# ORNL/DDStore

Hardware: NVIDIA H100
Metric: batch_fetch_GBps (higher is better)
Workload: dtype u8

## Files before the change

### ddstore_b200/csrc/kernels.cu

```cuda
#include <cuda_runtime.h>
#include <stdint.h>
#include <stdio.h>
#include <stdlib.h>
#include <string.h>

#include <algorithm>
#include <atomic>
#include <type_traits>

#include "kernels.h"

namespace {

thread_local char g_cuda_err[512] = "";
std::atomic<unsigned long long> g_launches{0};

#define CUDA_TRY(expr)                                                                                   \
    do {                                                                                                 \
        cudaError_t e__ = (expr);                                                                        \
        if (e__ != cudaSuccess) {                                                                        \
            snprintf(g_cuda_err, sizeof(g_cuda_err), "%s failed: %s (%s:%d)", #expr, cudaGetErrorString(e__), \
                     __FILE__, __LINE__);                                                                \
            return (int)e__ ? (int)e__ : -1;                                                             \
        }                                                                                                \
// ... 216 lines not shown
        if (code) {
            report(status, tag, idx[k], code);
            continue;
        }
        src[k] = s;
        nbytes[k] = count[k] * vp[k]->row_bytes;
    }
}

__device__ __forceinline__ int64_t warp_incl_scan(int64_t v, int lane) {
#pragma unroll
    for (int d = 1; d < 32; d <<= 1) {
        int64_t o = __shfl_up_sync(0xffffffffu, v, d);
        if (lane >= d) v += o;
    }
    return v;
}
__device__ __forceinline__ int64_t warp_sum(int64_t v) {
#pragma unroll
    for (int d = 16; d > 0; d >>= 1) v += __shfl_xor_sync(0xffffffffu, v, d);
    return v;
}

struct GatherArgs {
    ddsk_var_t var;
    const int64_t *starts;
    int64_t count;
    const uint64_t *req_src;
    const int64_t *req_dst;
    const uint32_t *seg_tab;
    PlanSrc plan;
    int64_t *total_out;
    int64_t nreq;
    char *dst;
    int64_t dst_cap;
    int64_t *offsets_out;
    unsigned long long *status;
    unsigned long long status_tag;
    unsigned int *counters;
    union {
        struct {
            char *mdst[DDSK_MAX_MULTI];
            int64_t mcap[DDSK_MAX_MULTI];
            int64_t *moffsets[DDSK_MAX_MULTI];
        };
        struct {
            int64_t pad_slot;
            uint64_t pad_bits;
            int pad_log2, pad_in_log2, pad_out_log2;
            int64_t *pad_lengths;
        };
    };
    int min_seg_chunks;
    int overlap, skip_wait;
    int wait1_valid, wait2_valid;
    unsigned int seq;
    unsigned int *ovl;
    int wait_plan;
    unsigned long long *plan_word;
    int64_t plan_tiles;
    unsigned int *tickets;
    unsigned long long *host_mirror;
    unsigned long long *dbg;
    const ddsk_push_t *push;
    int64_t push_nreq;
    unsigned long long push_step;
};

constexpr int64_t SEG_GRAIN = 16384;

struct Piece {
    uint64_t src;
    int64_t dpos;
    uint32_t n;
    uint32_t off;
};

template <int PCAP>
struct PlanView {
    uint32_t src_s, dst_s;
    __device__ __forceinline__ uint64_t s(int64_t i) const { return lds64(src_s + (uint32_t)i * 8u); }
    __device__ __forceinline__ int64_t d(int64_t i) const { return (int64_t)lds32(dst_s + (uint32_t)i * 4u); }
};
template <>
struct PlanView<0> {
    const uint64_t *src;
    const int64_t *dst;
    const uint32_t *seg_tab;
    __device__ __forceinline__ uint64_t s(int64_t i) const { return __ldcg(&src[i]); }
    __device__ __forceinline__ int64_t d(int64_t i) const { return __ldcg(&dst[i]); }
};

__device__ __forceinline__ void pad_lookup(const GatherArgs &a, int64_t idx, uint64_t &src, int64_t &payload) {
    const int64_t ix[1] = {idx};
    uint64_t s[1];
    int64_t nbytes[1];
    plan_many<1>(a.var, a.plan, ix, a.nreq, a.status, a.status_tag, s, nbytes);
    src = s[0];
    payload = min(nbytes[0], a.pad_slot);
}

__device__ __forceinline__ uint4 pad_pattern(uint64_t bits, int el) {
    uint32_t lo, hi;
    if (el == 0) lo = hi = (uint32_t)(bits & 0xFFu) * 0x01010101u;
    else if (el == 1) lo = hi = (uint32_t)(bits & 0xFFFFu) * 0x00010001u;
    else if (el == 2) lo = hi = (uint32_t)bits;
// ... 849 lines not shown
                over |= endv - vbase[v] > a.mcap[v];
            }
        if (PCAP > 0) over |= w.T > 0xFFFFFFFFll;
        if constexpr (CVT) {
            w.valign = true;
#pragma unroll
            for (int v = 0; v < DDSK_MAX_MULTI; v++) w.vb[v] = vbase[v];
        }
    }
    auto dst_of = [&](int64_t dpos) -> char * {
        if (FIXED && push) {
            int p = 0;
            for (int k = 1; k < w.push_n; k++)
                if (dpos >= push_rbase[k] * w.nb) p = k;
            return (char *)push_win[p] + push_dst_off + (dpos - push_rbase[p] * w.nb);
        }
        if (!multi) return a.dst + dpos;
        int64_t b = vbase[0];
        char *d = a.mdst[0];
#pragma unroll
        for (int k = 1; k < DDSK_MAX_MULTI; k++)
            if (dpos >= vbase[k]) {
                b = vbase[k];
                d = a.mdst[k];
            }
        return d + (dpos - b);
    };
    auto out_of = [&](int64_t dpos, int &code, uint32_t &lut) -> char * {
        if constexpr (CVT) {
            if (!multi) {
                code = code0;
                lut = lut_s + (uint32_t)c.lut_off[0];
                return a.dst + cvt_scale<NORM>(dpos, code0);
            }
            int64_t b = vbase[0];
            char *d = a.mdst[0];
            int cd = c.code[0], lo = c.lut_off[0];
#pragma unroll
            for (int k = 1; k < DDSK_MAX_MULTI; k++)
                if (dpos >= vbase[k]) {
                    b = vbase[k];
                    d = a.mdst[k];
                    cd = c.code[k];
                    lo = c.lut_off[k];
                }
            code = cd;
            lut = lut_s + (uint32_t)lo;
            return d + cvt_scale<NORM>(dpos - b, cd);
        } else {
            return nullptr;
        }
    };
    {
        if constexpr (PAD) {
            w.seg_bytes = ddsk_fixed_seg_bytes(w.T, w.nb, nwarps, a.min_seg_chunks, CH);
        } else {
        int64_t target = w.T / (nwarps * 8);
        const int64_t unit = (!FIXED && PCAP == 0) ? SEG_GRAIN : (int64_t)CH;
        target = max((int64_t)a.min_seg_chunks * CH, min(target, (int64_t)1 << 20));
        target = max(target, unit);
        if (FIXED && w.nb > 0 && w.nb <= target)
            w.seg_bytes = (target / w.nb) * w.nb;
        else
            w.seg_bytes = (target / unit) * unit;
        }
        w.nseg = w.T > 0 ? (w.T + w.seg_bytes - 1) / w.seg_bytes : 0;
    }
    if (over) {
        if (gwarp == 0 && lane == 0) report(a.status, a.status_tag, a.nreq, DDSK_CODE_CAPACITY);
        w.nseg = 0;
    }

    if (FIXED && !PAD && !push && (w.nb <= 0 || over)) {
        for (int64_t i = gwarp * 32 + lane; i < a.nreq; i += nwarps * 32) {
            uint64_t s;
            int code = dev_locate(a.var, a.starts[i], a.count, &s);
            if (code) report(a.status, a.status_tag, i, code);
        }
    }

    const uint32_t ring = smem_u32(smem_dyn) + (uint32_t)warp * (uint32_t)(S * STAGE);

    uint32_t issued = 0, consumed = 0;
    bool more = w.nseg > 0;
    while (true) {
        while (more && issued - consumed < (uint32_t)(S - 1)) {
            Piece pc;
            const uint32_t total = w.template next_group<STAGE>(a, lane, pc, pass_gate);
            if (total == 0) {
                more = false;
                break;
            }
            const uint32_t st = issued % S;
            const uint32_t bar = smem_u32(&full_bar[warp][st]);
            bulk_wait_read<1>();
            if (lane == 0) mbar_expect_tx(bar, total);
            __syncwarp();
            const uint32_t al = (uint32_t)(pc.src & 15u);
            desc[warp][st][lane].dpos = pc.dpos;
            desc[warp][st][lane].n = pc.n;
            desc[warp][st][lane].pack = pc.off | (al << 16);
            if (pc.n)
                tma_load_1d(ring + st * STAGE + pc.off, (const void *)(pc.src - al), (al + pc.n + 15u) & ~15u, bar);
            issued++;
        }
        if (consumed == issued) break;
        const uint32_t st = consumed % S;
        const uint32_t parity = (consumed / S) & 1u;
// ... 27 lines not shown
            const bool direct = my_code == 0 && my_n != 0 && (((uint32_t)(uint64_t)my_dst | my_n | (my_pack >> 16)) & 15u) == 0;
            if (direct) tma_store_1d(my_dst, ring + st * STAGE + (my_pack & 0xffffu), my_n);
            unsigned todo = __ballot_sync(0xffffffffu, my_n != 0 && !direct);
            while (todo) {
                const int j = __ffs(todo) - 1;
                todo &= todo - 1;
                const int64_t dpos = __shfl_sync(0xffffffffu, my_dpos, j);
                const uint32_t n = __shfl_sync(0xffffffffu, my_n, j);
                const uint32_t pk = __shfl_sync(0xffffffffu, my_pack, j);
                int code;
                uint32_t lut;
                char *const d = out_of(dpos, code, lut);
                const uint32_t s0 = ring + st * STAGE + (pk & 0xffffu);
                if constexpr (NORM) {
                    if (DDSK_CVT_IS_NORM(code)) {
                        norm_piece(c, multi, vbase, dpos, code, lut, d, s0 + (pk >> 16), n, lane);
                        continue;
                    }
                }
                switch (code) {
                case DDSK_CVT_F32_BF16: cvt_drain<DDSK_CVT_F32_BF16>(s0 + (pk >> 16), d, n, lut, lane); break;
                case DDSK_CVT_F32_F16: cvt_drain<DDSK_CVT_F32_F16>(s0 + (pk >> 16), d, n, lut, lane); break;
                case DDSK_CVT_F64_F32: cvt_drain<DDSK_CVT_F64_F32>(s0 + (pk >> 16), d, n, lut, lane); break;
                case DDSK_CVT_U8_LUT16: cvt_drain<DDSK_CVT_U8_LUT16>(s0 + (pk >> 16), d, n, lut, lane); break;
                case DDSK_CVT_U8_LUT32: cvt_drain<DDSK_CVT_U8_LUT32>(s0 + (pk >> 16), d, n, lut, lane); break;
                default: drain_chunk<CH>(s0, pk >> 16, d, n, lane); break;
                }
            }
        } else {
        char *const my_dst = dst_of(my_dpos);
        const bool direct = my_n != 0 && (((uint32_t)(uint64_t)my_dst | my_n | (my_pack >> 16)) & 15u) == 0;
        if (direct) tma_store_1d(my_dst, ring + st * STAGE + (my_pack & 0xffffu), my_n);
        unsigned todo = __ballot_sync(0xffffffffu, my_n != 0 && !direct);
        while (todo) {
            const int j = __ffs(todo) - 1;
            todo &= todo - 1;
            const int64_t dpos = __shfl_sync(0xffffffffu, my_dpos, j);
            const uint32_t n = __shfl_sync(0xffffffffu, my_n, j);
            const uint32_t pk = __shfl_sync(0xffffffffu, my_pack, j);
            drain_chunk<CH>(ring + st * STAGE + (pk & 0xffffu), pk >> 16, dst_of(dpos), n, lane);
        }
        }
        bulk_commit();
        __syncwarp();
        consumed++;
    }
    if (a.overlap || (FIXED && push)) {
        bulk_wait_all<0>();
        fence_proxy_async_global();
    } else {
        bulk_wait_read<0>();
    }
    __syncwarp();
    pass_gate();
    if (multi) {
        for (int64_t i = gwarp * 32 + lane; i < a.nreq + a.plan.nvars; i += nwarps * 32) {
            const int v = (int)(i / (a.plan.per_var + 1));
            const int64_t j = i - (int64_t)v * (a.plan.per_var + 1);
            if (v < a.plan.nvars && a.moffsets[v]) {
                const int64_t basev = w.pv.d((int64_t)v * a.plan.per_var);
                int64_t e = (v * a.plan.per_var + j == a.nreq) ? w.T : w.pv.d((int64_t)v * a.plan.per_var + j);
                if constexpr (CVT) a.moffsets[v][j] = cvt_scale<NORM>(e - basev, c.code[v]);
                else a.moffsets[v][j] = e - basev;
            }
        }
        if constexpr (CVT) {
            if (gwarp == 0 && lane == 0 && a.total_out) {
                int64_t t = 0;
#pragma unroll
                for (int v = 0; v < DDSK_MAX_MULTI; v++)
                    if (v < a.plan.nvars) t += cvt_scale<NORM>((v + 1 < a.plan.nvars ? vbase[v + 1] : w.T) - vbase[v], c.code[v]);
                *a.total_out = t;
            }
        }
    }
    if constexpr (PAD) {
        if (a.pad_lengths || w.nb == 0) {
            for (int64_t i = gwarp * 32 + lane; i < a.nreq; i += nwarps * 32) {
                uint64_t src;
                int64_t payload;
                pad_lookup(a, i, src, payload);
                if (a.pad_lengths) a.pad_lengths[i] = payload / a.var.row_bytes;
            }
        }
    }
    if (FIXED && a.offsets_out && !push) {
        if constexpr (CVT) {
            for (int64_t i = gwarp * 32 + lane; i <= a.nreq; i += nwarps * 32) a.offsets_out[i] = cvt_scale<NORM>(i * w.nb, code0);
        } else {
            for (int64_t i = gwarp * 32 + lane; i <= a.nreq; i += nwarps * 32) a.offsets_out[i] = i * w.nb;
        }
    }

    if (a.dbg && lane == 0) atomicMax(&a.dbg[blockIdx.x * 4 + 3], (unsigned long long)globaltimer_ns());
    if (a.overlap) {
        if (lane == 0) {
            __threadfence();
            const unsigned int slot = a.seq & 3u;
            const unsigned int done = atomicAdd(&a.ovl[slot], 1u);
            if (done == (unsigned int)(nwarps - 1)) {
                a.ovl[slot] = 0;
                a.ovl[8 + slot] = 0;
                if (a.wait_plan) a.plan_word[slot] = 0;
                if (a.wait1_valid) spin_until_done(a.ovl, a.seq - 1u, a.status, a.status_tag, a.nreq);
                __threadfence();
                st_release_u32(&a.ovl[4 + slot], a.seq);
            }
        }
    } else if (lane == 0) {
        if (FIXED && push) __threadfence_system(); else __threadfence();
        unsigned int done = atomicAdd(&a.counters[1], 1u);
        if (done == (unsigned int)(nwarps - 1)) {
            a.counters[0] = 0;
            a.counters[1] = 0;
            __threadfence();
            if (FIXED && push) {
                const ddsk_push_t *ps = a.push;
                for (int r = 0; r < ps->nranks; r++)
                    st_release_sys_u64((unsigned long long *)ps->win[r] + 8 + ps->me, a.push_step);
                const unsigned long long *hdr = (const unsigned long long *)ps->win[ps->me];
                const uint64_t t0 = globaltimer_ns();
                for (int r = 0; r < ps->nranks; r++)
                    while (ld_acquire_sys_u64(&hdr[8 + r]) < a.push_step) {
                        __nanosleep(200);
                        if (globaltimer_ns() - t0 > 30000000000ull) {
                            report(a.status, a.status_tag, a.nreq, DDSK_CODE_WATCHDOG);
                            __trap();
                        }
                    }
                const unsigned long long st = *(volatile const unsigned long long *)&hdr[3];
                if (st != DDSK_STATUS_OK) atomicMin(a.status, st | a.status_tag);
            }
            if (a.host_mirror) {
                a.host_mirror[0] = *(volatile unsigned long long *)a.status;
                a.host_mirror[1] = (unsigned long long)w.T;
                __threadfence_system();
            }
        }
    }
}

__global__ void __launch_bounds__(256) dds_small_get_kernel(const __grid_constant__ ddsk_var_t var, int64_t start, int64_t count,
                                                            char *__restrict__ dst, int64_t dst_cap,
                                                            volatile unsigned long long *flag, unsigned long long ticket) {
    uint64_t src = 0;
    const int code = dev_locate(var, start, count, &src);
    const int64_t n = code ? 0 : count * var.row_bytes;
    unsigned long long st = DDSK_STATUS_OK;
    if (code) st = (unsigned long long)code;
    else if (n > dst_cap) st = ((unsigned long long)1 << 8) | DDSK_CODE_CAPACITY;
    if (st == DDSK_STATUS_OK && n > 0) {
        const char *s = (const char *)src;
        if ((((uint64_t)s | (uint64_t)dst | (uint64_t)n) & 15u) == 0) {
            const uint4 *s4 = (const uint4 *)s;
            uint4 *d4 = (uint4 *)dst;
            for (int64_t i = threadIdx.x; i < (n >> 4); i += blockDim.x) d4[i] = s4[i];
        } else if ((((uint64_t)s | (uint64_t)dst | (uint64_t)n) & 3u) == 0) {
            const uint32_t *s1 = (const uint32_t *)s;
            uint32_t *d1 = (uint32_t *)dst;
            for (int64_t i = threadIdx.x; i < (n >> 2); i += blockDim.x) d1[i] = s1[i];
        } else {
            for (int64_t i = threadIdx.x; i < n; i += blockDim.x) dst[i] = s[i];
        }
    }
    __threadfence_system();
// ... 296 lines not shown
}

int geometry_for(bool fixed, int64_t request_bytes) {
    if (fixed) {
        if (g_geom_fixed_env >= 0) return g_geom_fixed_env;
        return request_bytes < 2048 ? kGeomSmall : kGeomLarge;
    }
    return g_geom_var_env >= 0 ? g_geom_var_env : kGeomVar;
}
int geometry_s_for(int64_t nreq) {
    if (nreq > kPlanSmemMax || nreq > g_plan_smem_default) return -1;
    if (g_geom_s_env >= 0 && kGeomsS[g_geom_s_env].pcap >= nreq) return g_geom_s_env;
    return nreq <= 4096 ? 0 : 1;
}

constexpr int smem_bytes_of(int nw, int s, int ch, int pcap) { return nw * s * (ch + 32) + (pcap ? pcap * 12 + 16 : 0); }
int static_smem_of(int nw, int s) { return nw * s * (8 + 32 * 16) + 16 * 8 + 64; }
int ctas_per_sm_for(int nw, int s, int ch, int pcap) {
    int per_sm = g_ctas_per_sm;
    while (per_sm > 1 && per_sm * (smem_bytes_of(nw, s, ch, pcap) + static_smem_of(nw, s) + 1024) > 227 * 1024) per_sm--;
    return per_sm;
}

bool cvt_has_norm(const ddsk_cvt_t *cvt) {
    for (int v = 0; v < DDSK_MAX_MULTI; v++)
        if (DDSK_CVT_IS_NORM(cvt->code[v])) return true;
    return false;
}

template <bool FIXED, int NW, int S, int CH, int PCAP, bool CVT = false, bool NORM = false, bool PAD = false>
int launch_gather_t(const GatherArgs &args_in, cudaStream_t stream, const ddsk_cvt_t *cvt = nullptr) {
    const int smem = smem_bytes_of(NW, S, CH, PCAP) + (CVT ? cvt->lut_bytes : 0);
    static std::atomic<unsigned long long> configured{0};
    auto kern = dds_gather_kernel<FIXED, NW, S, CH, PCAP, CVT, NORM, PAD>;
    int dev = 0;
    CUDA_TRY(cudaGetDevice(&dev));
    if (CVT) {
        if (dev >= 64 || !(configured.load() & (1ull << dev))) {
            cudaFuncAttributes fa;
            int optin = 0;
            CUDA_TRY(cudaFuncGetAttributes(&fa, kern));
            CUDA_TRY(cudaDeviceGetAttribute(&optin, cudaDevAttrMaxSharedMemoryPerBlockOptin, dev));
            const int most = std::min(smem_bytes_of(NW, S, CH, PCAP) + DDSK_MAX_MULTI * 1024, optin - (int)fa.sharedSizeBytes);
            CUDA_TRY(cudaFuncSetAttribute(kern, cudaFuncAttributeMaxDynamicSharedMemorySize, most));
            if (dev < 64) configured.fetch_or(1ull << dev);
        }
    } else if (dev >= 64 || !(configured.load() & (1ull << dev))) {
        CUDA_TRY(cudaFuncSetAttribute(kern, cudaFuncAttributeMaxDynamicSharedMemorySize, smem));
        if (dev < 64) configured.fetch_or(1ull << dev);
    }
    const int per_sm = ctas_per_sm_for(NW, S, CH, PCAP);
    GatherArgs args = args_in;
    args.dbg = g_dbg ? g_dbg + (size_t)(args.overlap ? (args.seq & 1u) : 0u) * kDbgRegion : nullptr;
    cudaLaunchConfig_t cfg = {};
    cfg.gridDim = dim3((unsigned)(g_sms * per_sm));
    cfg.blockDim = dim3(NW * 32);
    cfg.dynamicSmemBytes = smem;
    cfg.stream = stream;
    cudaLaunchAttribute attr[1];
    attr[0].id = cudaLaunchAttributeProgrammaticStreamSerialization;
    attr[0].val.programmaticStreamSerializationAllowed = g_pdl ? 1 : 0;
    cfg.attrs = attr;
    cfg.numAttrs = 1;
    if constexpr (CVT) {
        CUDA_TRY(cudaLaunchKernelEx(&cfg, kern, args, *cvt));
    } else {
        CUDA_TRY(cudaLaunchKernelEx(&cfg, kern, args, NoCvt{0}));
    }
    g_launches++;
    return 0;
}

template <int NW, int S, int CH, int PCAP>
bool cvt_s_fits_t(int lut_bytes) {
    cudaFuncAttributes fa;
    int dev = 0, optin = 0;
    if (cudaGetDevice(&dev) != cudaSuccess || cudaFuncGetAttributes(&fa, dds_gather_kernel<false, NW, S, CH, PCAP, true>) != cudaSuccess ||
        cudaDeviceGetAttribute(&optin, cudaDevAttrMaxSharedMemoryPerBlockOptin, dev) != cudaSuccess) {
        (void)cudaGetLastError();
        return false;
    }
    return smem_bytes_of(NW, S, CH, PCAP) + lut_bytes + (int)fa.sharedSizeBytes <= optin;
}

thread_local const void *g_l2_base = nullptr;
thread_local size_t g_l2_bytes = 0;

template <typename... KArgs, typename... Args>
int launch_pdl(void (*kern)(KArgs...), dim3 grid, dim3 block, cudaStream_t st, Args... args) {
    cudaLaunchConfig_t cfg = {};
    cfg.gridDim = grid;
    cfg.blockDim = block;
    cfg.dynamicSmemBytes = 0;
    cfg.stream = st;
    cudaLaunchAttribute attr[2];
    attr[0].id = cudaLaunchAttributeProgrammaticStreamSerialization;
    attr[0].val.programmaticStreamSerializationAllowed = g_pdl ? 1 : 0;
    cfg.attrs = attr;
    cfg.numAttrs = 1;
    if (g_l2_base && g_l2_bytes && g_l2_persist) {
        attr[1].id = cudaLaunchAttributeAccessPolicyWindow;
        attr[1].val.accessPolicyWindow.base_ptr = const_cast<void *>(g_l2_base);
        attr[1].val.accessPolicyWindow.num_bytes = g_l2_bytes;
        attr[1].val.accessPolicyWindow.hitRatio = 1.0f;
        attr[1].val.accessPolicyWindow.hitProp = cudaAccessPropertyPersisting;
        attr[1].val.accessPolicyWindow.missProp = cudaAccessPropertyStreaming;
        cfg.numAttrs = 2;
    }
// ... 372 lines not shown
```

### ddstore_b200/csrc/kernels.h

```cpp
#ifndef DDSK_KERNELS_H
#define DDSK_KERNELS_H

#include <stdint.h>

#ifdef __cplusplus
extern "C" {
#endif

#define DDSK_MAX_RANKS 64
#define DDSK_MAX_MULTI 4

typedef struct ddsk_var {
    const void *bases[DDSK_MAX_RANKS];
    int64_t lenlist[DDSK_MAX_RANKS];
    int64_t row_bytes;
    int32_t nranks;
    int32_t pad_;
} ddsk_var_t;

#define DDSK_STATUS_OK 0xFFFFFFFFFFFFFFFFull
#define DDSK_STATUS_ORD_SHIFT 48
#define DDSK_STATUS_REQ_MASK 0xFFFFFFFFFFull
#define DDSK_CODE_START 2
#define DDSK_CODE_COUNT 3
// ... 45 lines not shown
#define DDSK_CVT_PLAIN_IN_LOG2(c) ((c) == DDSK_CVT_F64_F32 ? 3 : ((c) == DDSK_CVT_F32_BF16 || (c) == DDSK_CVT_F32_F16) ? 2 : 0)
#define DDSK_CVT_PLAIN_OUT_LOG2(c) ((c) == DDSK_CVT_NONE ? 0 : ((c) == DDSK_CVT_F64_F32 || (c) == DDSK_CVT_U8_LUT32) ? 2 : 1)
#define DDSK_CVT_IN_LOG2(c) \
    (DDSK_CVT_IS_NORM(c) ? ((c) == DDSK_CVT_NORM_F64_F32 ? 3 : (c) >= DDSK_CVT_NORM_U8_F32 ? 0 : 2) : DDSK_CVT_PLAIN_IN_LOG2(c))
#define DDSK_CVT_OUT_LOG2(c)                                                                                              \
    (DDSK_CVT_IS_NORM(c) ? (((c) == DDSK_CVT_NORM_F32_F32 || (c) == DDSK_CVT_NORM_F64_F32 || (c) == DDSK_CVT_NORM_U8_F32) ? 2 : 1) \
                         : DDSK_CVT_PLAIN_OUT_LOG2(c))
typedef struct ddsk_cvt {
    int32_t code[DDSK_MAX_MULTI];
    int32_t lut_off[DDSK_MAX_MULTI];
    int32_t lut_bytes;
    int32_t pad_;
    uint32_t lut[DDSK_MAX_MULTI * 256];
    const float *norm[DDSK_MAX_MULTI];
    int32_t nchan[DDSK_MAX_MULTI];
    int32_t inner[DDSK_MAX_MULTI];
} ddsk_cvt_t;

int ddsk_gather_fixed(const ddsk_var_t *var, const int64_t *starts_dev, int64_t count, int64_t nreq, void *dst_dev,
                      int64_t dst_capacity, int64_t *offsets_dev_or_null, const ddsk_scratch_t *scr, int flags,
                      const ddsk_cvt_t *cvt, void *stream);

typedef struct ddsk_index {
    const int64_t *starts, *counts;
    const int64_t *sample_ids;
    const int64_t *table;
    int64_t nsamples;
} ddsk_index_t;

int ddsk_gather_var(const ddsk_var_t *var, const ddsk_index_t *index, int64_t nreq, void *dst_dev,
                    int64_t dst_capacity, int64_t *offsets_dev_or_null, ddsk_scratch_t *scr, int flags,
                    const ddsk_cvt_t *cvt, void *stream);
int ddsk_var_uses_scratch(int64_t nreq, int64_t dst_capacity, const ddsk_cvt_t *cvt);
int64_t ddsk_plan_smem_max(void);

int ddsk_gather_padded(const ddsk_var_t *var, const ddsk_index_t *index, int64_t nreq, int64_t max_rows, uint64_t pad_bits,
                       int pad_log2, int64_t *lengths, void *dst_dev, const ddsk_scratch_t *scr, int flags,
                       const ddsk_cvt_t *cvt, void *stream);

#if defined(__CUDACC__)
#define DDSK_HD __host__ __device__
#else
#define DDSK_HD
#endif

static inline DDSK_HD int64_t ddsk_fixed_seg_bytes(int64_t T, int64_t nb, int64_t nwarps, int64_t min_chunks, int64_t ch) {
    int64_t target = T / (nwarps * 8);
    if (target > ((int64_t)1 << 20)) target = (int64_t)1 << 20;
    if (target < min_chunks * ch) target = min_chunks * ch;
    if (target < ch) target = ch;
    return (nb > 0 && nb <= target) ? (target / nb) * nb : (target / ch) * ch;
}

typedef struct ddsk_pad_cut {
    int64_t pay_src, pay_len;
    int64_t pay_dst;
    int64_t pad_dst, pad_len;
} ddsk_pad_cut_t;
static inline DDSK_HD ddsk_pad_cut_t ddsk_pad_cut(int64_t i, int64_t payload, int64_t slot, int64_t lo, int64_t hi,
                                                  int in_log2, int out_log2) {
    ddsk_pad_cut_t c;
    const int64_t base = i * slot;
    const int64_t pe = payload < hi ? payload : hi;
    const int64_t ps = lo < pe ? lo : pe;
    const int64_t qs = lo > payload ? lo : payload;
    c.pay_src = base + ps;
    c.pay_len = pe - ps;
    c.pay_dst = ((base + ps) >> in_log2) << out_log2;
    c.pad_dst = ((base + qs) >> in_log2) << out_log2;
    c.pad_len = qs < hi ? ((hi - qs) >> in_log2) << out_log2 : 0;
    return c;
}

typedef struct ddsk_multi {
    int nvars;
    const ddsk_var_t *vars_dev;
    const int64_t *table[DDSK_MAX_MULTI];
    int64_t nsamples[DDSK_MAX_MULTI];
    void *dst[DDSK_MAX_MULTI];
    int64_t cap[DDSK_MAX_MULTI];
    int64_t *offsets[DDSK_MAX_MULTI];
} ddsk_multi_t;
int ddsk_gather_multi(const ddsk_multi_t *m, const int64_t *sample_ids_dev, int64_t nreq, ddsk_scratch_t *scr, int flags,
                      const ddsk_cvt_t *cvt, void *stream);

#define DDSK_PUSH_HDR_BYTES 4096
typedef struct ddsk_push {
    int32_t nranks, me;
    unsigned char *win[DDSK_MAX_RANKS];
    int64_t idx_off[2], dst_off[2];
    int64_t max_requests, max_bytes;
} ddsk_push_t;
int ddsk_gather_push(const ddsk_var_t *var, const ddsk_push_t *push_host, const ddsk_push_t *push_dev,
                     const int64_t *starts_dev, int64_t count, int64_t nreq, unsigned long long step,
                     const ddsk_scratch_t *scr, void *stream);

int ddsk_small_get(const ddsk_var_t *var, int64_t start, int64_t count, void *dst, int64_t dst_capacity,
                   unsigned long long *flag_dev, unsigned long long ticket, void *stream);

int ddsk_synth_fill(void *base_dev, int64_t first_global_row, int64_t nrows, int64_t disp, int itemsize, uint64_t seed,
                    void *stream);

typedef struct ddsk_mailbox {
    unsigned long long seq_head;
    int64_t start, count;
    uint64_t dst;
// ... 33 lines not shown
```

### ddstore_b200/csrc/store.cpp

```cpp
#include <cuda_runtime_api.h>
#include <sched.h>
#include <sys/random.h>
#include <unistd.h>

#include <algorithm>
#include <atomic>
#include <condition_variable>
#include <mutex>
#include <thread>
#include <cstdio>
#include <cstdlib>
#include <cstring>
#include <ctime>
#include <map>
#include <set>
#include <string>
#include <vector>

#include "ddstore_b200.h"
#include "internal.h"
#include "kernels.h"
#include "vmm.h"


// ... 1053 lines not shown
        if ((spins & 0xFFFF) == 0xFFFF) {
            cudaError_t q = cudaStreamQuery(s->db_stream);
            if (q != cudaErrorNotReady && q != cudaSuccess) {
                s->db_alive = false;
                return cuda_fail(q, "doorbell kernel");
            }
        }
#if defined(__x86_64__)
        __builtin_ia32_pause();
#endif
    }
    std::atomic_thread_fence(std::memory_order_acquire);
    const int code = (int)(r & 0xFFu);
    const int64_t n = code ? 0 : (count > 0 ? count * v->kv.row_bytes : 0);
    if (!dst_dev && n > 0) memcpy(dst, s->h_small + kSmallIdx * 16, (size_t)n);
    if (total_bytes) *total_bytes = n;
    if (!code) {
        if (bad_index) *bad_index = -1;
        return DDS_OK;
    }
    return decode_status_word(code == DDSK_CODE_CAPACITY ? (((unsigned long long)1 << 8) | DDSK_CODE_CAPACITY)
                                                          : (unsigned long long)code, bad_index);
}

static int small_get(dds_store_t *s, Var *v, int64_t start, int64_t count, void *dst, int64_t cap, bool dst_dev,
                     int64_t *total_bytes, int64_t *bad_index) {
    if (s->db_enabled && v->id >= 0) return doorbell_get(s, v, start, count, dst, cap, dst_dev, total_bytes, bad_index);
    cudaStream_t st = s->stream;
    volatile unsigned long long *flag = s->h_status;
    const unsigned long long ticket = ++s->small_ticket;
    void *d_dst = dst_dev ? dst : (void *)(s->d_small + kSmallIdx * 16);
    if (ddsk_small_get(&v->kv, start, count, d_dst, cap, s->scr.host_mirror, ticket, st))
        return fail(DDS_ERR_CUDA, ddsk_last_cuda_error());
    for (unsigned spins = 0; flag[2] != ticket; spins++) {
        if ((spins & 0x3FFF) == 0x3FFF) {
            cudaError_t q = cudaStreamQuery(st);
            if (q != cudaErrorNotReady) {
                if (q != cudaSuccess) return cuda_fail(q, "dds_small_get_kernel");
                if (flag[2] != ticket) return fail(DDS_ERR_CUDA, "small get: the kernel finished without publishing its ticket");
            }
        }
#if defined(__x86_64__)
        __builtin_ia32_pause();
#endif
    }
    std::atomic_thread_fence(std::memory_order_acquire);
    const unsigned long long stw = flag[0];
    const int64_t n = (int64_t)flag[1];
    if (!dst_dev && stw == DDSK_STATUS_OK && n > 0) memcpy(dst, s->h_small + kSmallIdx * 16, (size_t)n);
    if (total_bytes) *total_bytes = n;
    return decode_status_word(stw, bad_index);
}

static int stage_indices(dds_store_t *s, const int64_t *starts, const int64_t *counts, int64_t nreq, bool idx_dev,
                         cudaStream_t st, const int64_t **d_starts, const int64_t **d_counts) {
    if (idx_dev) return DDS_OK;
    if (nreq <= kSmallIdx) {
        int64_t *hs = (int64_t *)s->h_small, *hc = hs + kSmallIdx;
        memcpy(hs, starts, (size_t)nreq * 8);
        *d_starts = (const int64_t *)s->d_small;
        if (counts) {
            memcpy(hc, counts, (size_t)nreq * 8);
            *d_counts = (const int64_t *)s->d_small + kSmallIdx;
        }
        return DDS_OK;
    }
    if (int rc = ensure_idx(s, nreq)) return rc;
    CU(cudaMemcpyAsync(s->d_starts, starts, (size_t)nreq * 8, cudaMemcpyHostToDevice, st));
    *d_starts = s->d_starts;
    if (counts) {
        CU(cudaMemcpyAsync(s->d_counts, counts, (size_t)nreq * 8, cudaMemcpyHostToDevice, st));
        *d_counts = s->d_counts;
    }
    return DDS_OK;
}

static int batch_impl(dds_store_t *s, Var *v, bool by_sample, const int64_t *starts, const int64_t *counts,
                      int64_t fixed_count, int64_t nreq, void *dst, int64_t dst_capacity, int64_t *dst_offsets,
                      unsigned flags, void *cuda_stream, int64_t *total_bytes, int64_t *bad_index,
                      const ddsk_cvt_t *cvt = nullptr) {
    if (nreq < 0 || dst_capacity < 0) return fail(DDS_ERR_ARG, "negative nreq or capacity");
    if (nreq > 0 && !starts) return fail(DDS_ERR_ARG, "null starts / sample ids");
    const bool idx_dev = flags & DDS_IDX_ON_DEVICE, dst_dev = flags & DDS_DST_ON_DEVICE;
    const bool no_sync = flags & DDS_NO_SYNC;
    if (no_sync && !(idx_dev && dst_dev)) return fail(DDS_ERR_ARG, "async batches need device indices and a device destination");
    CU(cudaSetDevice(s->device));
    cudaStream_t st = cuda_stream ? (cudaStream_t)cuda_stream : s->stream;
    const bool chain = s->pending && no_sync && st == s->pending_stream;
    if (s->pending && !chain) {
        if (int rc = drain_pending(s)) return rc;
    }
    const int64_t R = v->kv.row_bytes;
    const bool fixed = !by_sample && counts == nullptr;
    const int64_t rows = v->lenlist.empty() ? 0 : v->lenlist.back();
    auto req_bytes = [&](int64_t c) { return c > 0 && c <= rows ? c * R : (int64_t)0; };
    const int64_t nb_fixed = fixed ? req_bytes(fixed_count) : 0;

    if (nreq == 0) {
        if (dst_offsets) {
            int64_t z = 0;
            if (dst_dev) CU(cudaMemcpyAsync(dst_offsets, &z, 8, cudaMemcpyHostToDevice, st));
            else dst_offsets[0] = 0;
            if (dst_dev) CU(cudaStreamSynchronize(st));
        }
        note_empty_async(s, no_sync);
        return DDS_OK;
    }

    if (fixed && nreq == 1 && !idx_dev && !no_sync && !cuda_stream && !dst_offsets && !cvt) {
        const int64_t need = nb_fixed;
        if (need <= (dst_dev ? (int64_t)(1 << 20) : kSmallOut) && (dst || need == 0))
            return small_get(s, v, starts[0], fixed_count, dst, dst_dev ? dst_capacity : std::min(dst_capacity, kSmallOut), dst_dev,
                             total_bytes, bad_index);
    }

    const int64_t *d_starts = starts, *d_counts = counts;
    if (int rc = stage_indices(s, starts, !fixed && !by_sample ? counts : nullptr, nreq, idx_dev, st, &d_starts, &d_counts))
        return rc;

    int64_t upper = -1;
    if (fixed)
        upper = sat_mul(nreq, nb_fixed);
    else if (!idx_dev && !by_sample) {
        upper = 0;
        for (int64_t i = 0; i < nreq; i++) upper = sat_add(upper, req_bytes(counts[i]));
    } else if (!idx_dev && by_sample && !v->h_tab_count.empty()) {
        upper = 0;
        for (int64_t i = 0; i < nreq; i++) {
            const int64_t id = starts[i];
            if (id >= 0 && id < v->nsamples) upper = sat_add(upper, req_bytes(v->h_tab_count[(size_t)id]));
        }
    }

    void *d_dst = dst;
    int64_t cap = dst_capacity;
    bool small_out = false;
    if (!dst_dev) {
        int64_t need = upper >= 0 ? std::min(upper, dst_capacity) : dst_capacity;
        if (need <= kSmallOut) {
// ... 782 lines not shown
```

### ddstore_b200/store.py

```python
import ctypes as C

import numpy as np

from . import _capi
from .comm import as_dds_comm

_NP_OK = {np.dtype(np.int32), np.dtype(np.int64), np.dtype(np.uint8), np.dtype(np.float32),
          np.dtype(np.float64), np.dtype(np.bool_)}
_TORCH_OK = {"torch.int32", "torch.int64", "torch.uint8", "torch.float32", "torch.float64", "torch.bool"}
_TORCH_HALF = {"torch.bfloat16", "torch.float16"}

_CVT_CODES = {("float32", "bfloat16"): _capi.CVT_F32_BF16, ("float32", "float16"): _capi.CVT_F32_F16,
              ("float64", "float32"): _capi.CVT_F64_F32, ("uint8", "bfloat16"): _capi.CVT_U8_LUT16,
              ("uint8", "float16"): _capi.CVT_U8_LUT16, ("uint8", "float32"): _capi.CVT_U8_LUT32}
_NORM_CODES = {("float32", "float32"): _capi.CVT_NORM_F32_F32, ("float32", "bfloat16"): _capi.CVT_NORM_F32_BF16,
               ("float32", "float16"): _capi.CVT_NORM_F32_F16, ("float64", "float32"): _capi.CVT_NORM_F64_F32,
               ("uint8", "float32"): _capi.CVT_NORM_U8_F32, ("uint8", "bfloat16"): _capi.CVT_NORM_U8_BF16,
               ("uint8", "float16"): _capi.CVT_NORM_U8_F16}
_U8_NORM = (_capi.CVT_NORM_U8_F32, _capi.CVT_NORM_U8_BF16, _capi.CVT_NORM_U8_F16)
_default_luts = {}


def _dtype_name(dt):
    s = str(dt)
# ... 70 lines not shown
    elif dtype.is_floating_point:
        v = float(value)
        t = torch.tensor([v], dtype=dtype)
        if math.isfinite(v) and not bool(torch.isfinite(t).all()):
            raise ValueError(f"pad_value {value!r} overflows {dtype}")
    else:
        if isinstance(value, float) and not value.is_integer():
            raise ValueError(f"pad_value {value!r} is not an integer ({dtype})")
        iv, info = int(value), torch.iinfo(dtype)
        if not info.min <= iv <= info.max:
            raise ValueError(f"pad_value {value!r} is outside the range of {dtype}")
        t = torch.tensor([iv], dtype=dtype)
    n = t.element_size()
    return int(t.view(getattr(torch, _INT_VIEW[n])).item()) & ((1 << (8 * n)) - 1)


def _lut_bits(t):
    import torch
    t = t.detach().reshape(-1).cpu().contiguous()
    return t.view(torch.int16 if t.element_size() == 2 else torch.int32).numpy().copy()


class _Buf:

    def __init__(self, arr, writable=False, half_ok=False):
        self.keep = arr
        if isinstance(arr, np.ndarray):
            assert arr.flags.c_contiguous
            if arr.dtype not in _NP_OK:
                raise NotImplementedError
            self.ptr, self.on_device = arr.ctypes.data, 0
            self.shape, self.itemsize, self.size = arr.shape, arr.dtype.itemsize, arr.size
        elif hasattr(arr, "data_ptr") and hasattr(arr, "element_size"):
            assert arr.is_contiguous()
            if str(arr.dtype) not in _TORCH_OK and not (half_ok and str(arr.dtype) in _TORCH_HALF):
                raise NotImplementedError
            self.ptr, self.on_device = arr.data_ptr(), 1 if arr.is_cuda else 0
            self.shape, self.itemsize, self.size = tuple(arr.shape), arr.element_size(), arr.numel()
        elif hasattr(arr, "__cuda_array_interface__"):
            cai = arr.__cuda_array_interface__
            if cai.get("strides") is not None:
                raise ValueError("device array must be C-contiguous")
            dt = np.dtype(cai["typestr"])
            if dt not in _NP_OK:
                raise NotImplementedError
            self.ptr, self.on_device = cai["data"][0], 1
            self.shape, self.itemsize = tuple(cai["shape"]), dt.itemsize
            self.size = int(np.prod(self.shape, dtype=np.int64))
        else:
            raise TypeError(f"unsupported array type {type(arr).__name__}")
        self.nbytes = self.size * self.itemsize


class _DevMem:

    def __init__(self, ptr, nbytes):
        self.__cuda_array_interface__ = {"shape": (int(nbytes),), "typestr": "|u1", "data": (int(ptr), False), "version": 2}


def _i64(x):
    return np.ascontiguousarray(x, dtype=np.int64)


class PyDDStore:
    def __init__(self, comm=None, method=0, device=None):
        self._L = _capi.lib()
        self._comm = as_dds_comm(comm)
        self._h = self._L.dds_create(self._comm.handle, -1 if device is None else int(device), int(method))
        if not self._h:
            raise RuntimeError(_capi.last_error())
        self.rank, self.size = self._L.dds_rank(self._h), self._L.dds_size(self._h)
        self._itemsize = {}
        self._cname = {}
        self._rowbytes = {}
        self.last_bad_index = -1

    def add(self, name, arr):
        b = _Buf(arr)
        nrows = b.shape[0]
        disp = b.size // b.shape[0] if b.shape[0] else int(np.prod(b.shape[1:], dtype=np.int64))
        _capi.raise_for(self._L.dds_add(self._h, name.encode(), b.ptr, nrows, disp, b.itemsize, b.on_device))

    def get(self, name, arr, start=0):
        cn = self._cname.get(name)
        if cn is None:
            cn = self._cname[name] = name.encode()
        if type(arr) is np.ndarray:
            assert arr.flags.c_contiguous
            if arr.dtype not in _NP_OK:
                raise NotImplementedError
            rc = self._L.dds_get(self._h, cn, int(start), arr.shape[0], arr.dtype.itemsize, arr.ctypes.data, 0)
        else:
            b = _Buf(arr, writable=True)
            rc = self._L.dds_get(self._h, cn, int(start), b.shape[0], b.itemsize, b.ptr, b.on_device)
        if rc:
            _capi.raise_for(rc)

    def epoch_begin(self):
        _capi.raise_for(self._L.dds_epoch_begin(self._h))

    def epoch_end(self):
        _capi.raise_for(self._L.dds_epoch_end(self._h))

    def free(self):
        if self._h:
            self._itemsize.clear()
            _capi.raise_for(self._L.dds_free(self._h))

    def init(self, name, nrows, disp, itemsize=1):
        _capi.raise_for(self._L.dds_init(self._h, name.encode(), int(nrows), int(disp), int(itemsize)))

    def update(self, name, arr, offset, stream=None, wait=True):
        b = _Buf(arr)
        if wait:
            rc = self._L.dds_update(self._h, name.encode(), b.ptr, b.shape[0], int(offset), b.itemsize, b.on_device)
        else:
            rc = self._L.dds_update_async(self._h, name.encode(), b.ptr, b.shape[0], int(offset), b.itemsize,
                                          b.on_device, self._stream_arg(stream))
        _capi.raise_for(rc)

    def ingest(self, name, arr, offset):
        b = _Buf(arr)
        if b.on_device:
            raise ValueError("ingest takes host arrays (use update for device arrays)")
        _capi.raise_for(self._L.dds_ingest(self._h, name.encode(), b.ptr, b.shape[0], int(offset), b.itemsize))

    def ingest_wait(self):
        _capi.raise_for(self._L.dds_ingest_wait(self._h))

    def get_batch(self, name, starts, counts=None, out=None, count=None, offsets=None, stream=None, wait=True,
                  overlap=False, src_dtype=None, lut=None, normalize=False, pad_rows=None, pad_value=0, lengths=None):
        if out is None:
            raise ValueError("get_batch needs an `out` buffer (like get(), it never allocates)")
        if pad_rows is not None:
            if counts is None:
                raise ValueError("pad_rows needs counts (there is no fixed-count padded batch)")
            if count is not None or offsets is not None:
                raise ValueError("a padded batch takes neither `count` nor `offsets`")
        cv = lut_keep = None
        if normalize and src_dtype is None:
            raise ValueError("normalize=True needs src_dtype")
        if src_dtype is not None:
            cv, lut_keep = _conversion(src_dtype, getattr(out, "dtype", None), lut, normalize)
        else:
            itemsize = self._itemsize.get(name)
            if itemsize is None:
                itemsize = self._itemsize[name] = self.query(name)["itemsize"]
        ob = _Buf(out, writable=True, half_ok=cv is not None or pad_rows is not None)
        s_dev = hasattr(starts, "data_ptr") and getattr(starts, "is_cuda", False)
        if s_dev:
            nreq = starts.numel()
            sp = starts.data_ptr()
            cp = counts.data_ptr() if counts is not None else None
            keep = (starts, counts)
        else:
            sa = _i64(starts)
            nreq = sa.size
            sp = sa.ctypes.data
            ca = _i64(counts) if counts is not None else None
            cp = ca.ctypes.data if ca is not None else None
            keep = (sa, ca)
        flags = (_capi.IDX_ON_DEVICE if s_dev else 0) | (_capi.DST_ON_DEVICE if ob.on_device else 0)
        if not wait:
            flags |= _capi.NO_SYNC | (_capi.OVERLAP if overlap else 0)
        if pad_rows is not None:
            return self._padded(name, False, sp, cp, nreq, out, ob, cv, pad_rows, pad_value, lengths, flags, stream,
                                (keep, lut_keep))
        op = None
        if offsets is not None:
            fb = _Buf(offsets, writable=True)
            if fb.on_device != ob.on_device or fb.itemsize != 8 or fb.size < nreq + 1:
                raise ValueError("offsets must be int64[len(starts)+1] with the same residency as out")
            op = fb.ptr
        total, bad = C.c_int64(0), C.c_int64(-1)
        if cv is None:
            rc = self._L.dds_get_batch(self._h, name.encode(), sp, cp, 1 if count is None else int(count), nreq,
                                       itemsize, ob.ptr, ob.nbytes, op, flags,
                                       self._stream_arg(stream), C.byref(total), C.byref(bad))
        else:
            rc = self._L.dds_get_batch_convert(self._h, name.encode(), sp, cp, 1 if count is None else int(count), nreq,
                                               ob.ptr, ob.nbytes, op, flags, self._stream_arg(stream), C.byref(cv),
                                               C.byref(total), C.byref(bad))
        del keep, lut_keep
        self.last_bad_index = bad.value
# ... 208 lines not shown
```

Baseline: 1466.

## Right-size fixed-batch grid, per-CTA completion counting, and a fast Python path

For fixed-count batches the host now works out the segment size and a reduced CTA count from the batch shape and passes the segment size to the kernel, so small batches no longer launch a full grid. The completion counter is now bumped once per CTA after a __syncthreads rather than once per warp, and only warps that have tail work pass the gate. The host side skips redundant cudaSetDevice calls, and the Python get_batch gains a fast path for async device batches that bypasses argument validation. The risks are correctness of the gate and counter logic with fewer CTAs, and a fast path that does less validation.

After: 1469, median of 6. Within noise of the previous version (+0.2%).

```diff
diff --git a/ddstore_b200/csrc/kernels.cu b/ddstore_b200/csrc/kernels.cu
--- a/ddstore_b200/csrc/kernels.cu
+++ b/ddstore_b200/csrc/kernels.cu
@@ -292,6 +292,7 @@
         };
     };
     int min_seg_chunks;
+    int64_t fixed_seg;
     int overlap, skip_wait;
     int wait1_valid, wait2_valid;
     unsigned int seq;
@@ -1247,8 +1248,8 @@
         }
     };
     {
-        if constexpr (PAD) {
-            w.seg_bytes = ddsk_fixed_seg_bytes(w.T, w.nb, nwarps, a.min_seg_chunks, CH);
+        if (FIXED && !push) {
+            w.seg_bytes = a.fixed_seg;
         } else {
         int64_t target = w.T / (nwarps * 8);
         const int64_t unit = (!FIXED && PCAP == 0) ? SEG_GRAIN : (int64_t)CH;
@@ -1382,7 +1383,13 @@
         bulk_wait_read<0>();
     }
     __syncwarp();
-    pass_gate();
+    {
+        bool tail = false;
+        if (multi) tail = gwarp * 32 < a.nreq + a.plan.nvars;
+        if (PAD && a.pad_lengths) tail = gwarp * 32 < a.nreq;
+        if (FIXED && a.offsets_out && !push) tail = gwarp * 32 <= a.nreq;
+        if (tail) pass_gate();
+    }
     if (multi) {
         for (int64_t i = gwarp * 32 + lane; i < a.nreq + a.plan.nvars; i += nwarps * 32) {
             const int v = (int)(i / (a.plan.per_var + 1));
@@ -1423,12 +1430,15 @@
     }
 
     if (a.dbg && lane == 0) atomicMax(&a.dbg[blockIdx.x * 4 + 3], (unsigned long long)globaltimer_ns());
+    __syncthreads();
+    if (warp != 0) return;
+    if (a.overlap) pass_gate();
     if (a.overlap) {
         if (lane == 0) {
             __threadfence();
             const unsigned int slot = a.seq & 3u;
             const unsigned int done = atomicAdd(&a.ovl[slot], 1u);
-            if (done == (unsigned int)(nwarps - 1)) {
+            if (done == gridDim.x - 1u) {
                 a.ovl[slot] = 0;
                 a.ovl[8 + slot] = 0;
                 if (a.wait_plan) a.plan_word[slot] = 0;
@@ -1440,7 +1450,7 @@
     } else if (lane == 0) {
         if (FIXED && push) __threadfence_system(); else __threadfence();
         unsigned int done = atomicAdd(&a.counters[1], 1u);
-        if (done == (unsigned int)(nwarps - 1)) {
+        if (done == gridDim.x - 1u) {
             a.counters[0] = 0;
             a.counters[1] = 0;
             __threadfence();
@@ -1843,8 +1853,18 @@
     const int per_sm = ctas_per_sm_for(NW, S, CH, PCAP);
     GatherArgs args = args_in;
     args.dbg = g_dbg ? g_dbg + (size_t)(args.overlap ? (args.seq & 1u) : 0u) * kDbgRegion : nullptr;
+    int ctas = g_sms * per_sm;
+    if (FIXED && !args.push) {
+        int64_t nb = PAD ? args.pad_slot
+                         : (args.count <= args.var.lenlist[args.var.nranks - 1] && args.count > 0 ? args.count * args.var.row_bytes : 0);
+        int64_t T = nb > 0 && args.nreq <= INT64_MAX / nb ? nb * args.nreq : 0;
+        if (T > args.dst_cap) T = 0;
+        const ddsk_fixed_shape_t sh = ddsk_fixed_shape(T, nb, args.nreq, NW, ctas, args.min_seg_chunks, CH);
+        args.fixed_seg = sh.seg_bytes;
+        ctas = sh.ctas;
+    }
     cudaLaunchConfig_t cfg = {};
-    cfg.gridDim = dim3((unsigned)(g_sms * per_sm));
+    cfg.gridDim = dim3((unsigned)ctas);
     cfg.blockDim = dim3(NW * 32);
     cfg.dynamicSmemBytes = smem;
     cfg.stream = stream;
diff --git a/ddstore_b200/csrc/kernels.h b/ddstore_b200/csrc/kernels.h
--- a/ddstore_b200/csrc/kernels.h
+++ b/ddstore_b200/csrc/kernels.h
@@ -121,6 +121,25 @@
     return (nb > 0 && nb <= target) ? (target / nb) * nb : (target / ch) * ch;
 }
 
+typedef struct ddsk_fixed_shape {
+    int64_t seg_bytes, nseg;
+    int32_t ctas, pad_;
+} ddsk_fixed_shape_t;
+static inline DDSK_HD ddsk_fixed_shape_t ddsk_fixed_shape(int64_t T, int64_t nb, int64_t nreq, int64_t nw, int64_t full_ctas,
+                                                          int64_t min_chunks, int64_t ch) {
+    ddsk_fixed_shape_t s;
+    s.seg_bytes = ddsk_fixed_seg_bytes(T, nb, full_ctas * nw, min_chunks, ch);
+    s.nseg = T > 0 ? (T + s.seg_bytes - 1) / s.seg_bytes : 0;
+    int64_t warps = (nreq + 1 + 1023) / 1024;
+    if (warps < s.nseg) warps = s.nseg;
+    int64_t ctas = (warps + nw - 1) / nw;
+    if (ctas > full_ctas) ctas = full_ctas;
+    if (ctas < 1) ctas = 1;
+    s.ctas = (int32_t)ctas;
+    s.pad_ = 0;
+    return s;
+}
+
 typedef struct ddsk_pad_cut {
     int64_t pay_src, pay_len;
     int64_t pay_dst;
diff --git a/ddstore_b200/csrc/store.cpp b/ddstore_b200/csrc/store.cpp
--- a/ddstore_b200/csrc/store.cpp
+++ b/ddstore_b200/csrc/store.cpp
@@ -1129,6 +1129,12 @@
     return decode_status_word(stw, bad_index);
 }
 
+static cudaError_t use_device(int device) {
+    int cur = -1;
+    if (cudaGetDevice(&cur) == cudaSuccess && cur == device) return cudaSuccess;
+    return cudaSetDevice(device);
+}
+
 static int stage_indices(dds_store_t *s, const int64_t *starts, const int64_t *counts, int64_t nreq, bool idx_dev,
                          cudaStream_t st, const int64_t **d_starts, const int64_t **d_counts) {
     if (idx_dev) return DDS_OK;
@@ -1161,7 +1167,7 @@
     const bool idx_dev = flags & DDS_IDX_ON_DEVICE, dst_dev = flags & DDS_DST_ON_DEVICE;
     const bool no_sync = flags & DDS_NO_SYNC;
     if (no_sync && !(idx_dev && dst_dev)) return fail(DDS_ERR_ARG, "async batches need device indices and a device destination");
-    CU(cudaSetDevice(s->device));
+    CU(use_device(s->device));
     cudaStream_t st = cuda_stream ? (cudaStream_t)cuda_stream : s->stream;
     const bool chain = s->pending && no_sync && st == s->pending_stream;
     if (s->pending && !chain) {
diff --git a/ddstore_b200/store.py b/ddstore_b200/store.py
--- a/ddstore_b200/store.py
+++ b/ddstore_b200/store.py
@@ -146,6 +146,17 @@
         self.nbytes = self.size * self.itemsize
 
 
+_FAST_FLAGS = _capi.IDX_ON_DEVICE | _capi.DST_ON_DEVICE | _capi.NO_SYNC
+_FAST_FLAGS_OVL = _FAST_FLAGS | _capi.OVERLAP
+_FAST_DTYPE = {None: False}
+
+
+def _fast_dtype(arr):
+    dt = arr.dtype
+    ok = _FAST_DTYPE[dt] = hasattr(arr, "data_ptr") and hasattr(arr, "element_size") and str(dt) in _TORCH_OK
+    return ok
+
+
 class _DevMem:
 
     def __init__(self, ptr, nbytes):
@@ -224,6 +235,27 @@
 
     def get_batch(self, name, starts, counts=None, out=None, count=None, offsets=None, stream=None, wait=True,
                   overlap=False, src_dtype=None, lut=None, normalize=False, pad_rows=None, pad_value=0, lengths=None):
+        if (not wait and counts is None and offsets is None and src_dtype is None and pad_rows is None
+                and lengths is None and not normalize):
+            ok = _FAST_DTYPE.get(getattr(out, "dtype", None))
+            if ok is None:
+                ok = _fast_dtype(out)
+            if ok and getattr(out, "is_cuda", False) and getattr(starts, "is_cuda", False) and out.is_contiguous():
+                cn = self._cname.get(name)
+                if cn is None:
+                    cn = self._cname[name] = name.encode()
+                itemsize = self._itemsize.get(name)
+                if itemsize is None:
+                    itemsize = self._itemsize[name] = self.query(name)["itemsize"]
+                total, bad = C.c_int64(0), C.c_int64(-1)
+                rc = self._L.dds_get_batch(self._h, cn, starts.data_ptr(), None, 1 if count is None else int(count),
+                                           starts.numel(), itemsize, out.data_ptr(), out.numel() * out.element_size(), None,
+                                           _FAST_FLAGS_OVL if overlap else _FAST_FLAGS,
+                                           None if stream is None else (int(stream) or 1), C.byref(total), C.byref(bad))
+                self.last_bad_index = bad.value
+                if rc:
+                    _capi.raise_for(rc)
+                return total.value
         if out is None:
             raise ValueError("get_batch needs an `out` buffer (like get(), it never allocates)")
         if pad_rows is not None:
```
